# MalvinaNikandrou/mafed

Hardware: AMD Instinct MI355X
Metric: train samples/sec VLPythia-410M+MAFED, 256img+32txt tok, bs=32, 1/2/4/8 GPU (higher is better)
Workload: dtype bf16; 1 GPU; VLPythia-410m + MAFED distill step (student fwd+bwd, frozen-teacher fwd, replay CE, 23-layer per-modality MSE, clip 2.0, AdamW), 256 img + 32 txt tokens; global_batch=32, per_gpu_batch=32, seq_len=288, parallelism=dp1, random_init_weights=True

## Files before the change

mafed_amd/csrc/attn_mfma.hip:

```cpp
#include <type_traits>

#include "attn.h"

namespace mafed {

namespace {

typedef __attribute__((address_space(3))) bf16x4* lds_bf16x4_ptr;

template <int D>
__device__ __forceinline__ int swz(int row) {
  if (D == 64) return ((row >> 1) & 3) << 1;
  if (D == 128) return (row & 7) << 1;
  return ((row & 7) << 1) | ((row >> 3) & 1);
}
template <int D>
__device__ __forceinline__ int tile_off(int row, int chunk) {
  if (D == 64) return row * 128 + ((chunk ^ swz<64>(row)) << 4);
  if (D == 128) return row * 256 + ((chunk ^ swz<128>(row)) << 4);
  return row * 512 + ((chunk ^ (((row & 7) << 1) | ((row >> 3) & 1))) << 4);
}

__device__ __forceinline__ void unpack8(const uint4& v, float (&f)[8]) {
  f[0] = __uint_as_float(v.x << 16); f[1] = __uint_as_float(v.x & 0xffff0000u);
// ... 683 lines not shown
  extern __shared__ __attribute__((aligned(16))) char lds[];
  constexpr int NTH = NW * 64;
  const int tid = threadIdx.x, lane = tid & 63;
  const int wave = __builtin_amdgcn_readfirstlane(tid >> 6);
  const int S = sh.S, H = sh.H, rot = sh.rot, P = sh.P, T = sh.T;
  const int h = blockIdx.x, b = blockIdx.y;
  const int nrows = (S + 31) / 32 * 32;
  char* kimg = lds;
  char* vimg = lds + nrows * D * 2;
  float* kbias = reinterpret_cast<float*>(lds + 2 * nrows * D * 2);
  float* red = kbias + 2 * nrows;
  if (bsum && tid < D) red[tid] = 0.f;
  const int64_t rstride = (int64_t)H * 3 * D;
  const bf16_t* qb = qkv + ((int64_t)b * S * H + h) * 3 * D;
  const bf16_t* kb = qb + D;
  const bf16_t* vb = qb + 2 * D;
  const int64_t ostride = (int64_t)H * D;
  const bf16_t* ob = out + (int64_t)b * S * ostride + (int64_t)h * D;
  const bf16_t* dob = dout + (int64_t)b * S * ostride + (int64_t)h * D;
  const float* Lrow = lse + ((int64_t)b * H + h) * S;
  const int nslices = (S + 15) / 16;
  const int hc = rot >> 4, items = S * hc;
  dma_rows<D, NW>(kimg, kb, rstride, nrows, S, wave, lane);
  dma_rows<D, NW>(vimg, vb, rstride, nrows, S, wave, lane);
  RotPre pre[2];
#pragma unroll
  for (int u = 0; u < 2; ++u)
    if (tid + NTH * u < items) rot_pre_load(pre[u], tid + NTH * u, hc, rot, rc, rs);
  for (int k = tid; k < nrows; k += NTH) kbias[k] = key_ok(am, b, k, P, T, S) ? 0.f : -INFINITY;
  constexpr bool PREFETCH = NW == 4;
  ColRaw<D> qraw, doraw, oraw;
  float Lnext = 0.f;
  if (PREFETCH) {
    const int s0 = nslices - 1 - snake<NW>(wave, 0);
    if (s0 >= 0) {
      col_raw_issue<D, true>(qraw, qb, rstride, s0 * 16, S, rot, rc, rs, lane);
      col_raw_issue<D, false>(doraw, dob, ostride, s0 * 16, S, 0, rc, rs, lane);
      col_raw_issue<D, false>(oraw, ob, ostride, s0 * 16, S, 0, rc, rs, lane);
      const int q = s0 * 16 + (lane & 15);
      Lnext = q < S ? Lrow[q] : 0.f;
    }
  }
  wait_vm0();
  __syncthreads();
  rot_fix_rows<D, NTH>(kimg, items, hc, rot, rc, rs, pre, tid);
  __syncthreads();
  const int g = lane >> 4;
  const float scale = rsqrtf((float)D);
  const float scale2 = scale * MAFED_LOG2E;
  for (int t = 0;; ++t) {
    const int slice = nslices - 1 - snake<NW>(wave, t);
    if (slice < 0) break;
    const int q0 = slice * 16;
    const int myq = q0 + (lane & 15);
    if (!PREFETCH) {
      col_raw_issue<D, true>(qraw, qb, rstride, q0, S, rot, rc, rs, lane);
      col_raw_issue<D, false>(doraw, dob, ostride, q0, S, 0, rc, rs, lane);
      col_raw_issue<D, false>(oraw, ob, ostride, q0, S, 0, rc, rs, lane);
      Lnext = myq < S ? Lrow[myq] : 0.f;
    }
    bf16x8 qf[D / 32], dof[D / 32];
    col_raw_finish<D, true>(qf, qraw, q0, S, rot, lane);
    col_raw_finish<D, false>(dof, doraw, q0, S, 0, lane);
    const float L2 = Lnext * MAFED_LOG2E;
    float dl = 0.f;
    {
      bf16x8 of[D / 32];
      col_raw_finish<D, false>(of, oraw, q0, S, 0, lane);
      const int nxt = nslices - 1 - snake<NW>(wave, t + 1);
      if (PREFETCH && nxt >= 0) {
        col_raw_issue<D, true>(qraw, qb, rstride, nxt * 16, S, rot, rc, rs, lane);
        col_raw_issue<D, false>(doraw, dob, ostride, nxt * 16, S, 0, rc, rs, lane);
        col_raw_issue<D, false>(oraw, ob, ostride, nxt * 16, S, 0, rc, rs, lane);
        const int q = nxt * 16 + (lane & 15);
        Lnext = q < S ? Lrow[q] : 0.f;
      }
#pragma unroll
      for (int ks = 0; ks < D / 32; ++ks)
#pragma unroll
        for (int e = 0; e < 8; ++e) dl += (float)dof[ks][e] * (float)of[ks][e];
      dl = col_sum_sw(dl);
    }
    if (myq < S && g == 0) delta[((int64_t)b * H + h) * S + myq] = dl;
    f32x4 dq[D / 16];
#pragma unroll
    for (int i = 0; i < D / 16; ++i) dq[i] = (f32x4){0.f, 0.f, 0.f, 0.f};
    const int last_kt = (q0 + 15) / 64;
    auto tile = [&](const int kt, const int nj, auto mask_tag) {
      constexpr bool MASK = decltype(mask_tag)::value;
      f32x4 ds[4];
#pragma unroll
      for (int j = 0; j < 4; ++j) {
        ds[j] = (f32x4){0.f, 0.f, 0.f, 0.f};
        if (!MASK || j < nj) {
          f32x4 s = (f32x4){0.f, 0.f, 0.f, 0.f}, dp = (f32x4){0.f, 0.f, 0.f, 0.f};
#pragma unroll
          for (int ks = 0; ks < D / 32; ++ks) {
            s = __builtin_amdgcn_mfma_f32_16x16x32_bf16(frag_row<D>(kimg, kt * 4 + j, ks, lane), qf[ks], s, 0, 0, 0);
            dp = __builtin_amdgcn_mfma_f32_16x16x32_bf16(frag_row<D>(vimg, kt * 4 + j, ks, lane), dof[ks], dp, 0, 0, 0);
          }
          if (MASK) {
            const float4 kb4 = *reinterpret_cast<const float4*>(kbias + kt * 64 + j * 16 + 4 * g);
            const float kbv[4] = {kb4.x, kb4.y, kb4.z, kb4.w};
#pragma unroll
            for (int r = 0; r < 4; ++r) {
              const int key = kt * 64 + j * 16 + 4 * g + r;
              float x = s[r] * scale2 - L2 + kbv[r];
              x = key > myq ? -INFINITY : x;
              ds[j][r] = __builtin_amdgcn_exp2f(x) * (dp[r] - dl) * scale;
            }
          } else {
#pragma unroll
            for (int r = 0; r < 4; ++r) ds[j][r] = __builtin_amdgcn_exp2f(s[r] * scale2 - L2) * (dp[r] - dl) * scale;
          }
        }
      }
      const bf16x8 d0 = pack_acc(ds[0], ds[1]);
#pragma unroll
      for (int dt = 0; dt < D / 16; ++dt) dq[dt] = __builtin_amdgcn_mfma_f32_16x16x32_bf16(frag_tr<D>(kimg, dt, kt * 2, lane), d0, dq[dt], 0, 0, 0);
      if (!MASK || nj > 2) {
        const bf16x8 d1 = pack_acc(ds[2], ds[3]);
#pragma unroll
        for (int dt = 0; dt < D / 16; ++dt)
          dq[dt] = __builtin_amdgcn_mfma_f32_16x16x32_bf16(frag_tr<D>(kimg, dt, kt * 2 + 1, lane), d1, dq[dt], 0, 0, 0);
      }
    };
    const int kt_plain = last_kt < P / 64 ? last_kt : P / 64;
    for (int kt = 0; kt < kt_plain; ++kt) tile(kt, 4, std::false_type{});
    for (int kt = kt_plain; kt <= last_kt; ++kt) tile(kt, kt == last_kt ? ((q0 + 15 - kt * 64) >> 4) + 1 : 4, std::true_type{});
    bf16_t* dqp = dqkv + ((int64_t)b * S * H + h) * 3 * D + (int64_t)myq * rstride;
    store_grad_unrot<D>(dqp, dq, rot, rc, rs, myq, lane, myq < S);
    if (bsum) {
#pragma unroll
      for (int dt = 0; dt < D / 16; ++dt)
#pragma unroll
        for (int r = 0; r < 4; ++r) {
          const float v = row16_sum(myq < S ? dq[dt][r] : 0.f);
          if ((lane & 15) == 0) atomicAdd(red + dt * 16 + 4 * g + r, v);
        }
    }
  }
  if (bsum) {
    __syncthreads();
    if (tid < D) atomicAdd(bsum + (int64_t)h * 3 * D + tid, red[tid]);
  }
}

template <int D, int NW = 4>
__global__ __launch_bounds__(NW * 64, (D == 64 ? 2 : 1) * NW / 4) void attn_bwd_dkv_res_kernel(const bf16_t* __restrict__ qkv, const bf16_t* __restrict__ dout,
                                                               const float* __restrict__ lse, const float* __restrict__ delta, AttnShape sh,
                                                               const float* __restrict__ rc, const float* __restrict__ rs,
                                                               const int64_t* __restrict__ am, bf16_t* __restrict__ dqkv,
                                                               float* __restrict__ bsum) {
  extern __shared__ __attribute__((aligned(16))) char lds[];
  constexpr int NTH = NW * 64;
  const int tid = threadIdx.x, lane = tid & 63;
  const int wave = __builtin_amdgcn_readfirstlane(tid >> 6);
  const int S = sh.S, H = sh.H, rot = sh.rot, P = sh.P, T = sh.T;
  const int h = blockIdx.x, b = blockIdx.y;
  const int nrows = (S + 31) / 32 * 32;
  char* qimg = lds;
  char* doimg = lds + nrows * D * 2;
  float* L2s = reinterpret_cast<float*>(lds + 2 * nrows * D * 2);
  float* Ds = L2s + nrows;
  float* red = Ds + nrows;
  if (bsum && tid < 2 * D) red[tid] = 0.f;
  const int64_t rstride = (int64_t)H * 3 * D;
  const bf16_t* qb = qkv + ((int64_t)b * S * H + h) * 3 * D;
  const bf16_t* kb = qb + D;
  const bf16_t* vb = qb + 2 * D;
  const int64_t ostride = (int64_t)H * D;
  const bf16_t* dob = dout + (int64_t)b * S * ostride + (int64_t)h * D;
  const float* Lrow = lse + ((int64_t)b * H + h) * S;
  const float* Drow = delta + ((int64_t)b * H + h) * S;
  const int nslices = (S + 15) / 16;
  const int hc = rot >> 4, items = S * hc;
  dma_rows<D, NW>(qimg, qb, rstride, nrows, S, wave, lane);
  dma_rows<D, NW>(doimg, dob, ostride, nrows, S, wave, lane);
  RotPre pre[2];
#pragma unroll
  for (int u = 0; u < 2; ++u)
    if (tid + NTH * u < items) rot_pre_load(pre[u], tid + NTH * u, hc, rot, rc, rs);
  for (int q = tid; q < nrows; q += NTH) {
    L2s[q] = q < S ? Lrow[q] * MAFED_LOG2E : INFINITY;
    Ds[q] = q < S ? Drow[q] : 0.f;
  }
  ColRaw<D> kraw, vraw;
  {
    const int s0 = snake<NW>(wave, 0);
    if (s0 < nslices) {
      col_raw_issue<D, true>(kraw, kb, rstride, s0 * 16, S, rot, rc, rs, lane);
      col_raw_issue<D, false>(vraw, vb, rstride, s0 * 16, S, 0, rc, rs, lane);
    }
  }
  wait_vm0();
  __syncthreads();
  rot_fix_rows<D, NTH>(qimg, items, hc, rot, rc, rs, pre, tid);
  __syncthreads();
  const int g = lane >> 4;
  const float scale = rsqrtf((float)D);
  const float scale2 = scale * MAFED_LOG2E;
  const int nqt = (nrows + 63) / 64;
  for (int t = 0;; ++t) {
    const int slice = snake<NW>(wave, t);
    if (slice >= nslices) break;
    const int k0 = slice * 16;
    const int mykey = k0 + (lane & 15);
    const int mykey_eff = key_ok(am, b, mykey, P, T, S) ? mykey : 0x7fffffff;
    bf16x8 kf[D / 32], vf[D / 32];
    col_raw_finish<D, true>(kf, kraw, k0, S, rot, lane);
    col_raw_finish<D, false>(vf, vraw, k0, S, 0, lane);
    {
      const int nxt = snake<NW>(wave, t + 1);
      if (nxt < nslices) {
        col_raw_issue<D, true>(kraw, kb, rstride, nxt * 16, S, rot, rc, rs, lane);
        col_raw_issue<D, false>(vraw, vb, rstride, nxt * 16, S, 0, rc, rs, lane);
      }
    }
    f32x4 dk[D / 16], dv[D / 16];
#pragma unroll
    for (int i = 0; i < D / 16; ++i) { dk[i] = (f32x4){0.f, 0.f, 0.f, 0.f}; dv[i] = (f32x4){0.f, 0.f, 0.f, 0.f}; }
    const int qt0 = k0 / 64;
    const bool text_keys = k0 + 15 >= P;
    auto tile = [&](const int qt, const int jlo, const int jhi, auto edge_tag) {
      constexpr bool EDGE = decltype(edge_tag)::value;
      f32x4 p[4], ds[4];
#pragma unroll
      for (int j = 0; j < 4; ++j) {
        p[j] = (f32x4){0.f, 0.f, 0.f, 0.f};
        ds[j] = (f32x4){0.f, 0.f, 0.f, 0.f};
        if (!EDGE || (j >= jlo && j < jhi)) {
          f32x4 s = (f32x4){0.f, 0.f, 0.f, 0.f}, dp = (f32x4){0.f, 0.f, 0.f, 0.f};
#pragma unroll
          for (int ks = 0; ks < D / 32; ++ks) {
            s = __builtin_amdgcn_mfma_f32_16x16x32_bf16(frag_row<D>(qimg, qt * 4 + j, ks, lane), kf[ks], s, 0, 0, 0);
            dp = __builtin_amdgcn_mfma_f32_16x16x32_bf16(frag_row<D>(doimg, qt * 4 + j, ks, lane), vf[ks], dp, 0, 0, 0);
          }
          const float4 L4 = *reinterpret_cast<const float4*>(L2s + qt * 64 + j * 16 + 4 * g);
          const float4 D4 = *reinterpret_cast<const float4*>(Ds + qt * 64 + j * 16 + 4 * g);
          const float Lv[4] = {L4.x, L4.y, L4.z, L4.w}, Dv[4] = {D4.x, D4.y, D4.z, D4.w};
#pragma unroll
          for (int r = 0; r < 4; ++r) {
            float x = s[r] * scale2 - Lv[r];
            if (EDGE) {
              const int q = qt * 64 + j * 16 + 4 * g + r;
              x = mykey_eff > q ? -INFINITY : x;
            }
            const float pv = __builtin_amdgcn_exp2f(x);
            p[j][r] = pv;
            ds[j][r] = pv * (dp[r] - Dv[r]) * scale;
          }
        }
      }
      if (!EDGE || jlo < 2) {
        const bf16x8 p0 = pack_acc(p[0], p[1]), d0 = pack_acc(ds[0], ds[1]);
#pragma unroll
        for (int dt = 0; dt < D / 16; ++dt) {
          dv[dt] = __builtin_amdgcn_mfma_f32_16x16x32_bf16(frag_tr<D>(doimg, dt, qt * 2, lane), p0, dv[dt], 0, 0, 0);
          dk[dt] = __builtin_amdgcn_mfma_f32_16x16x32_bf16(frag_tr<D>(qimg, dt, qt * 2, lane), d0, dk[dt], 0, 0, 0);
        }
      }
      if (!EDGE || jhi > 2) {
        const bf16x8 p1 = pack_acc(p[2], p[3]), d1 = pack_acc(ds[2], ds[3]);
#pragma unroll
        for (int dt = 0; dt < D / 16; ++dt) {
          dv[dt] = __builtin_amdgcn_mfma_f32_16x16x32_bf16(frag_tr<D>(doimg, dt, qt * 2 + 1, lane), p1, dv[dt], 0, 0, 0);
          dk[dt] = __builtin_amdgcn_mfma_f32_16x16x32_bf16(frag_tr<D>(qimg, dt, qt * 2 + 1, lane), d1, dk[dt], 0, 0, 0);
        }
      }
    };
    const int nfull = nrows / 64;
    for (int qt = qt0; qt < nqt; ++qt) {
      const int jlo = qt == qt0 ? (k0 - qt * 64) >> 4 : 0;
      const int jhi = (nrows - qt * 64) >> 4 < 4 ? (nrows - qt * 64) >> 4 : 4;
      if (qt == qt0 || text_keys || qt >= nfull) tile(qt, jlo, jhi, std::true_type{});
      else tile(qt, 0, 4, std::false_type{});
    }
    bf16_t* dkp = dqkv + ((int64_t)b * S * H + h) * 3 * D + (int64_t)mykey * rstride + D;
    store_grad_unrot<D>(dkp, dk, rot, rc, rs, mykey, lane, mykey < S);
    if (mykey < S) {
      bf16_t* dvp = dkp + D;
#pragma unroll
      for (int dt = 0; dt < D / 16; ++dt) store4(dvp + dt * 16 + 4 * g, make_float4(dv[dt][0], dv[dt][1], dv[dt][2], dv[dt][3]));
    }
    if (bsum) {
#pragma unroll
      for (int dt = 0; dt < D / 16; ++dt)
#pragma unroll
        for (int r = 0; r < 4; ++r) {
          const float vk = row16_sum(mykey < S ? dk[dt][r] : 0.f), vv = row16_sum(mykey < S ? dv[dt][r] : 0.f);
          if ((lane & 15) == 0) {
            atomicAdd(red + dt * 16 + 4 * g + r, vk);
            atomicAdd(red + D + dt * 16 + 4 * g + r, vv);
          }
        }
    }
  }
  if (bsum) {
    __syncthreads();
    if (tid < 2 * D) atomicAdd(bsum + (int64_t)h * 3 * D + D + tid, red[tid]);
  }
}

static double attn_fwd_flops(const AttnShape& sh) { return 4.0 * sh.D * ((double)sh.S * (sh.S + 1) / 2.0) * sh.H * sh.B; }

static bool attn_resident_fits(const AttnShape& sh, size_t* bytes) {
  const size_t nrows = (size_t)(sh.S + 31) / 32 * 32;
  *bytes = nrows * sh.D * 2 * 2 + nrows * 4 * 2 + (size_t)sh.D * 4 * 2;
  return sh.D <= 128 && *bytes <= 160 * 1024;
}
static int g_attn_variant = 0;

template <typename K>
static void set_lds_attr(K kfn, size_t bytes) {
  (void)hipFuncSetAttribute((const void*)kfn, hipFuncAttributeMaxDynamicSharedMemorySize, (int)bytes);
}

int attn_mfma_fwd_launch(const void* qkv, const AttnShape& sh, const float* rc, const float* rs, const int64_t* am, void* out, float* lse,
                         hipStream_t st) {
  size_t bytes;
  if (g_attn_variant != 1 && attn_resident_fits(sh, &bytes)) {
    dim3 grid(sh.H, sh.B), block(attn_fwd_waves<64>() * 64);
    if (!sh.causal) {
      if (sh.D != 64) { set_error("attn_fwd (bidirectional, bf16): head_dim %d has no MFMA kernel (CLIP towers use 64)", sh.D); return MAFED_EINVAL; }
      set_lds_attr(attn_fwd_res_kernel<64, false>, bytes);
      launch(K_ATTN_FWD, 2.0 * attn_fwd_flops(sh), attn_fwd_res_kernel<64, false>, grid, block, bytes, st, (const bf16_t*)qkv, sh, rc, rs, am,
             (bf16_t*)out, lse);
      return MAFED_OK;
    }
    if (sh.D == 64) {
      set_lds_attr(attn_fwd_res_kernel<64>, bytes);
      launch(K_ATTN_FWD, attn_fwd_flops(sh), attn_fwd_res_kernel<64>, grid, block, bytes, st, (const bf16_t*)qkv, sh, rc, rs, am, (bf16_t*)out, lse);
    } else {
      set_lds_attr(attn_fwd_res_kernel<128>, bytes);
      launch(K_ATTN_FWD, attn_fwd_flops(sh), attn_fwd_res_kernel<128>, grid, dim3(attn_fwd_waves<128>() * 64), bytes, st, (const bf16_t*)qkv, sh, rc, rs, am, (bf16_t*)out, lse);
    }
    return MAFED_OK;
  }
  if (!sh.causal) { set_error("attn_fwd (bidirectional, bf16): S=%d D=%d does not fit the resident kernel", sh.S, sh.D); return MAFED_EINVAL; }
  dim3 grid((sh.S + 63) / 64, sh.H, sh.B), block(256);
  const size_t tb = (size_t)2 * 64 * sh.D * 2;
#define MAFED_FWD_TILED(DD)                                                                                                       \
  do {                                                                                                                            \
    set_lds_attr(attn_fwd_mfma_kernel<DD>, tb);                                                                                   \
    launch(K_ATTN_FWD, attn_fwd_flops(sh), attn_fwd_mfma_kernel<DD>, grid, block, tb, st, (const bf16_t*)qkv, sh, rc, rs, am, (bf16_t*)out, lse);                    \
  } while (0)
  if (sh.D == 64) MAFED_FWD_TILED(64);
  else if (sh.D == 128) MAFED_FWD_TILED(128);
  else MAFED_FWD_TILED(256);
#undef MAFED_FWD_TILED
  return MAFED_OK;
}

int attn_mfma_bwd_launch(const void* qkv, const void* out, const void* dout, const float* lse, const AttnShape& sh, const float* rc,
                         const float* rs, const int64_t* am, void* dqkv, float* delta, float* colsum, bool* colsum_done, hipStream_t st) {
  size_t bytes;
  *colsum_done = false;
  if (g_attn_variant != 1 && attn_resident_fits(sh, &bytes)) {
    dim3 grid(sh.H, sh.B), block(256);
    if (sh.D == 64) {
      set_lds_attr(attn_bwd_dq_res_kernel<64>, bytes);
      set_lds_attr(attn_bwd_dkv_res_kernel<64>, bytes);
      launch(K_ATTN_BWD_DQ, attn_fwd_flops(sh), attn_bwd_dq_res_kernel<64>, grid, block, bytes, st, (const bf16_t*)qkv, (const bf16_t*)out, (const bf16_t*)dout, lse, sh, rc, rs, am,
                                                             (bf16_t*)dqkv, delta, colsum);
      launch(K_ATTN_BWD_DKV, attn_fwd_flops(sh), attn_bwd_dkv_res_kernel<64>, grid, block, bytes, st, (const bf16_t*)qkv, (const bf16_t*)dout, lse, delta, sh, rc, rs, am, (bf16_t*)dqkv, colsum);
    } else {
      set_lds_attr(attn_bwd_dq_res_kernel<128>, bytes);
      set_lds_attr(attn_bwd_dkv_res_kernel<128>, bytes);
      launch(K_ATTN_BWD_DQ, attn_fwd_flops(sh), attn_bwd_dq_res_kernel<128>, grid, block, bytes, st, (const bf16_t*)qkv, (const bf16_t*)out, (const bf16_t*)dout, lse, sh, rc, rs, am,
                                                              (bf16_t*)dqkv, delta, colsum);
      launch(K_ATTN_BWD_DKV, attn_fwd_flops(sh), attn_bwd_dkv_res_kernel<128>, grid, block, bytes, st, (const bf16_t*)qkv, (const bf16_t*)dout, lse, delta, sh, rc, rs, am, (bf16_t*)dqkv, colsum);
    }
    *colsum_done = colsum != nullptr;
    return MAFED_OK;
  }
  dim3 grid((sh.S + 63) / 64, sh.H, sh.B), block(256);
  const size_t tb = (size_t)2 * 64 * sh.D * 2, tb2 = tb + 2 * 64 * 4;
#define MAFED_BWD_TILED(DD)                                                                                                       \
  do {                                                                                                                            \
    set_lds_attr(attn_bwd_dq_mfma_kernel<DD>, tb);                                                                                \
    set_lds_attr(attn_bwd_dkv_mfma_kernel<DD>, tb2);                                                                              \
    launch(K_ATTN_BWD_DQ, attn_fwd_flops(sh), attn_bwd_dq_mfma_kernel<DD>, grid, block, tb, st, (const bf16_t*)qkv, (const bf16_t*)out, (const bf16_t*)dout, lse, sh, rc, rs, am, \
                                                         (bf16_t*)dqkv, delta);                                                  \
    launch(K_ATTN_BWD_DKV, attn_fwd_flops(sh), attn_bwd_dkv_mfma_kernel<DD>, grid, block, tb2, st, (const bf16_t*)qkv, (const bf16_t*)dout, lse, delta, sh, rc, rs, am,   \
                                                           (bf16_t*)dqkv);                                                       \
  } while (0)
  if (sh.D == 64) MAFED_BWD_TILED(64);
  else if (sh.D == 128) MAFED_BWD_TILED(128);
  else MAFED_BWD_TILED(256);
#undef MAFED_BWD_TILED
  return MAFED_OK;
}

void attn_mfma_set_variant(int v) { g_attn_variant = v; }


}
```

Before: 1006 samples/s.

## Fuse attention backward dQ and dK/dV into one LDS-resident kernel

Adds a single backward attention kernel for head_dim 64. It loads Q, K, V and dO once into LDS per (head, batch), computes delta in-kernel, and interleaves key-slice (dK/dV) and query-slice (dQ) work items across 12 waves. This replaces the two separate resident kernels, which each reloaded tiles and recomputed S and dP. The cost is a larger LDS footprint, fewer blocks per CU, and S and dP still being recomputed in both the key and query items.

```diff
diff --git a/mafed_amd/csrc/attn_mfma.hip b/mafed_amd/csrc/attn_mfma.hip
--- a/mafed_amd/csrc/attn_mfma.hip
+++ b/mafed_amd/csrc/attn_mfma.hip
@@ -1009,12 +1009,256 @@
   }
 }
 
+constexpr int kFusedWaves = 12;
+
+__global__ __launch_bounds__(kFusedWaves * 64, kFusedWaves / 4) void attn_bwd_fused_kernel(const bf16_t* __restrict__ qkv, const bf16_t* __restrict__ out,
+                                                                             const bf16_t* __restrict__ dout, const float* __restrict__ lse, AttnShape sh,
+                                                                             const float* __restrict__ rc, const float* __restrict__ rs,
+                                                                             const int64_t* __restrict__ am, bf16_t* __restrict__ dqkv,
+                                                                             float* __restrict__ delta, float* __restrict__ bsum) {
+  constexpr int D = 64, NW = kFusedWaves, NTH = NW * 64;
+  extern __shared__ __attribute__((aligned(16))) char lds[];
+  const int tid = threadIdx.x, lane = tid & 63;
+  const int wave = __builtin_amdgcn_readfirstlane(tid >> 6);
+  const int S = sh.S, H = sh.H, rot = sh.rot, P = sh.P, T = sh.T;
+  const int h = blockIdx.x, b = blockIdx.y;
+  const int nrows = (S + 31) / 32 * 32;
+  char* qimg = lds;
+  char* kimg = lds + 1 * nrows * D * 2;
+  char* vimg = lds + 2 * nrows * D * 2;
+  char* doimg = lds + 3 * nrows * D * 2;
+  float* kbias = reinterpret_cast<float*>(lds + 4 * nrows * D * 2);
+  float* L2s = kbias + nrows;
+  float* Ds = L2s + nrows;
+  float* red = Ds + nrows;
+  if (bsum && tid < 3 * D) red[tid] = 0.f;
+  const int64_t rstride = (int64_t)H * 3 * D;
+  const bf16_t* qb = qkv + ((int64_t)b * S * H + h) * 3 * D;
+  const bf16_t* kb = qb + D;
+  const bf16_t* vb = qb + 2 * D;
+  const int64_t ostride = (int64_t)H * D;
+  const bf16_t* ob = out + (int64_t)b * S * ostride + (int64_t)h * D;
+  const bf16_t* dob = dout + (int64_t)b * S * ostride + (int64_t)h * D;
+  const float* Lrow = lse + ((int64_t)b * H + h) * S;
+  const int nslices = (S + 15) / 16;
+  const int hc = rot >> 4, items = S * hc;
+  dma_rows<D, NW>(qimg, qb, rstride, nrows, S, wave, lane);
+  dma_rows<D, NW>(doimg, dob, ostride, nrows, S, wave, lane);
+  dma_rows<D, NW>(kimg, kb, rstride, nrows, S, wave, lane);
+  dma_rows<D, NW>(vimg, vb, rstride, nrows, S, wave, lane);
+  RotPre pre[2];
+#pragma unroll
+  for (int u = 0; u < 2; ++u)
+    if (tid + NTH * u < items) rot_pre_load(pre[u], tid + NTH * u, hc, rot, rc, rs);
+  for (int k = tid; k < nrows; k += NTH) {
+    kbias[k] = key_ok(am, b, k, P, T, S) ? 0.f : -INFINITY;
+    L2s[k] = k < S ? Lrow[k] * MAFED_LOG2E : INFINITY;
+  }
+  for (int r0 = 0; r0 < nrows; r0 += NTH / 8) {
+    const int row = r0 + (tid >> 3), ch = tid & 7;
+    float dl = 0.f;
+    if (row < S) {
+      float fo[8], fd[8];
+      unpack8(*reinterpret_cast<const uint4*>(ob + (int64_t)row * ostride + ch * 8), fo);
+      unpack8(*reinterpret_cast<const uint4*>(dob + (int64_t)row * ostride + ch * 8), fd);
+#pragma unroll
+      for (int e = 0; e < 8; ++e) dl = fmaf(fd[e], fo[e], dl);
+    }
+    dl += __shfl_xor(dl, 1, 64);
+    dl += __shfl_xor(dl, 2, 64);
+    dl += __shfl_xor(dl, 4, 64);
+    if (row < nrows && ch == 0) {
+      Ds[row] = dl;
+      if (row < S) delta[((int64_t)b * H + h) * S + row] = dl;
+    }
+  }
+  wait_vm0();
+  __syncthreads();
+  rot_fix_rows<D, NTH>(qimg, items, hc, rot, rc, rs, pre, tid);
+  rot_fix_rows<D, NTH>(kimg, items, hc, rot, rc, rs, pre, tid);
+  __syncthreads();
+  const int g = lane >> 4;
+  const float scale = rsqrtf((float)D);
+  const float scale2 = scale * MAFED_LOG2E;
+  const int nqt = (nrows + 63) / 64;
+  const int nfull = nrows / 64;
+  bf16_t* dqkv_bh = dqkv + ((int64_t)b * S * H + h) * 3 * D;
+
+  auto key_item = [&](const int slice) {
+    const int k0 = slice * 16;
+    const int mykey = k0 + (lane & 15);
+    const int mykey_eff = key_ok(am, b, mykey, P, T, S) ? mykey : 0x7fffffff;
+    bf16x8 kf[D / 32], vf[D / 32];
+#pragma unroll
+    for (int ks = 0; ks < D / 32; ++ks) {
+      kf[ks] = frag_row<D>(kimg, slice, ks, lane);
+      vf[ks] = frag_row<D>(vimg, slice, ks, lane);
+    }
+    f32x4 dk[D / 16], dv[D / 16];
+#pragma unroll
+    for (int i = 0; i < D / 16; ++i) { dk[i] = (f32x4){0.f, 0.f, 0.f, 0.f}; dv[i] = (f32x4){0.f, 0.f, 0.f, 0.f}; }
+    const int qt0 = k0 / 64;
+    const bool text_keys = k0 + 15 >= P;
+    auto tile = [&](const int qt, const int jlo, const int jhi, auto edge_tag) {
+      constexpr bool EDGE = decltype(edge_tag)::value;
+#pragma nounroll
+      for (int hh = 0; hh < 2; ++hh) {
+        if (EDGE && (2 * hh + 1 < jlo || 2 * hh >= jhi)) continue;
+        f32x4 p[2], ds[2];
+#pragma unroll
+        for (int jj = 0; jj < 2; ++jj) {
+          const int j = 2 * hh + jj;
+          p[jj] = (f32x4){0.f, 0.f, 0.f, 0.f};
+          ds[jj] = (f32x4){0.f, 0.f, 0.f, 0.f};
+          if (!EDGE || (j >= jlo && j < jhi)) {
+            f32x4 s = (f32x4){0.f, 0.f, 0.f, 0.f}, dp = (f32x4){0.f, 0.f, 0.f, 0.f};
+#pragma unroll
+            for (int ks = 0; ks < D / 32; ++ks) {
+              s = __builtin_amdgcn_mfma_f32_16x16x32_bf16(frag_row<D>(qimg, qt * 4 + j, ks, lane), kf[ks], s, 0, 0, 0);
+              dp = __builtin_amdgcn_mfma_f32_16x16x32_bf16(frag_row<D>(doimg, qt * 4 + j, ks, lane), vf[ks], dp, 0, 0, 0);
+            }
+            const float4 L4 = *reinterpret_cast<const float4*>(L2s + qt * 64 + j * 16 + 4 * g);
+            const float4 D4 = *reinterpret_cast<const float4*>(Ds + qt * 64 + j * 16 + 4 * g);
+            const float Lv[4] = {L4.x, L4.y, L4.z, L4.w}, Dv[4] = {D4.x, D4.y, D4.z, D4.w};
+#pragma unroll
+            for (int r = 0; r < 4; ++r) {
+              float x = s[r] * scale2 - Lv[r];
+              if (EDGE) {
+                const int q = qt * 64 + j * 16 + 4 * g + r;
+                x = mykey_eff > q ? -INFINITY : x;
+              }
+              const float pv = __builtin_amdgcn_exp2f(x);
+              p[jj][r] = pv;
+              ds[jj][r] = pv * (dp[r] - Dv[r]) * scale;
+            }
+          }
+        }
+        const bf16x8 p0 = pack_acc(p[0], p[1]), d0 = pack_acc(ds[0], ds[1]);
+#pragma unroll
+        for (int dt = 0; dt < D / 16; ++dt) {
+          dv[dt] = __builtin_amdgcn_mfma_f32_16x16x32_bf16(frag_tr<D>(doimg, dt, qt * 2 + hh, lane), p0, dv[dt], 0, 0, 0);
+          dk[dt] = __builtin_amdgcn_mfma_f32_16x16x32_bf16(frag_tr<D>(qimg, dt, qt * 2 + hh, lane), d0, dk[dt], 0, 0, 0);
+        }
+      }
+    };
+    for (int qt = qt0; qt < nqt; ++qt) {
+      const int jlo = qt == qt0 ? (k0 - qt * 64) >> 4 : 0;
+      const int jhi = (nrows - qt * 64) >> 4 < 4 ? (nrows - qt * 64) >> 4 : 4;
+      if (qt == qt0 || text_keys || qt >= nfull) tile(qt, jlo, jhi, std::true_type{});
+      else tile(qt, 0, 4, std::false_type{});
+    }
+    bf16_t* dkp = dqkv_bh + (int64_t)mykey * rstride + D;
+    store_grad_unrot<D>(dkp, dk, rot, rc, rs, mykey, lane, mykey < S);
+    if (mykey < S) {
+      bf16_t* dvp = dkp + D;
+#pragma unroll
+      for (int dt = 0; dt < D / 16; ++dt) store4(dvp + dt * 16 + 4 * g, make_float4(dv[dt][0], dv[dt][1], dv[dt][2], dv[dt][3]));
+    }
+    if (bsum) {
+#pragma unroll
+      for (int dt = 0; dt < D / 16; ++dt)
+#pragma unroll
+        for (int r = 0; r < 4; ++r) {
+          const float vk = row16_sum(mykey < S ? dk[dt][r] : 0.f), vv = row16_sum(mykey < S ? dv[dt][r] : 0.f);
+          if ((lane & 15) == 0) {
+            atomicAdd(red + D + dt * 16 + 4 * g + r, vk);
+            atomicAdd(red + 2 * D + dt * 16 + 4 * g + r, vv);
+          }
+        }
+    }
+  };
+
+  auto query_item = [&](const int slice) {
+    const int q0 = slice * 16;
+    const int myq = q0 + (lane & 15);
+    bf16x8 qf[D / 32], dof[D / 32];
+#pragma unroll
+    for (int ks = 0; ks < D / 32; ++ks) {
+      qf[ks] = frag_row<D>(qimg, slice, ks, lane);
+      dof[ks] = frag_row<D>(doimg, slice, ks, lane);
+    }
+    const float L2 = L2s[myq], dl = Ds[myq];
+    f32x4 dq[D / 16];
+#pragma unroll
+    for (int i = 0; i < D / 16; ++i) dq[i] = (f32x4){0.f, 0.f, 0.f, 0.f};
+    const int last_kt = (q0 + 15) / 64;
+    auto tile = [&](const int kt, const int nj, auto mask_tag) {
+      constexpr bool MASK = decltype(mask_tag)::value;
+#pragma nounroll
+      for (int hh = 0; hh < 2; ++hh) {
+        if (MASK && 2 * hh >= nj) break;
+        f32x4 ds[2];
+#pragma unroll
+        for (int jj = 0; jj < 2; ++jj) {
+          const int j = 2 * hh + jj;
+          ds[jj] = (f32x4){0.f, 0.f, 0.f, 0.f};
+          if (!MASK || j < nj) {
+            f32x4 s = (f32x4){0.f, 0.f, 0.f, 0.f}, dp = (f32x4){0.f, 0.f, 0.f, 0.f};
+#pragma unroll
+            for (int ks = 0; ks < D / 32; ++ks) {
+              s = __builtin_amdgcn_mfma_f32_16x16x32_bf16(frag_row<D>(kimg, kt * 4 + j, ks, lane), qf[ks], s, 0, 0, 0);
+              dp = __builtin_amdgcn_mfma_f32_16x16x32_bf16(frag_row<D>(vimg, kt * 4 + j, ks, lane), dof[ks], dp, 0, 0, 0);
+            }
+            if (MASK) {
+              const float4 kb4 = *reinterpret_cast<const float4*>(kbias + kt * 64 + j * 16 + 4 * g);
+              const float kbv[4] = {kb4.x, kb4.y, kb4.z, kb4.w};
+#pragma unroll
+              for (int r = 0; r < 4; ++r) {
+                const int key = kt * 64 + j * 16 + 4 * g + r;
+                float x = s[r] * scale2 - L2 + kbv[r];
+                x = key > myq ? -INFINITY : x;
+                ds[jj][r] = __builtin_amdgcn_exp2f(x) * (dp[r] - dl) * scale;
+              }
+            } else {
+#pragma unroll
+              for (int r = 0; r < 4; ++r) ds[jj][r] = __builtin_amdgcn_exp2f(s[r] * scale2 - L2) * (dp[r] - dl) * scale;
+            }
+          }
+        }
+        const bf16x8 d0 = pack_acc(ds[0], ds[1]);
+#pragma unroll
+        for (int dt = 0; dt < D / 16; ++dt)
+          dq[dt] = __builtin_amdgcn_mfma_f32_16x16x32_bf16(frag_tr<D>(kimg, dt, kt * 2 + hh, lane), d0, dq[dt], 0, 0, 0);
+      }
+    };
+    const int kt_plain = last_kt < P / 64 ? last_kt : P / 64;
+    for (int kt = 0; kt < kt_plain; ++kt) tile(kt, 4, std::false_type{});
+    for (int kt = kt_plain; kt <= last_kt; ++kt) tile(kt, kt == last_kt ? ((q0 + 15 - kt * 64) >> 4) + 1 : 4, std::true_type{});
+    store_grad_unrot<D>(dqkv_bh + (int64_t)myq * rstride, dq, rot, rc, rs, myq, lane, myq < S);
+    if (bsum) {
+#pragma unroll
+      for (int dt = 0; dt < D / 16; ++dt)
+#pragma unroll
+        for (int r = 0; r < 4; ++r) {
+          const float v = row16_sum(myq < S ? dq[dt][r] : 0.f);
+          if ((lane & 15) == 0) atomicAdd(red + dt * 16 + 4 * g + r, v);
+        }
+    }
+  };
+
+  for (int t = 0;; ++t) {
+    const int item = snake<NW>(wave, t);
+    if (item >= 2 * nslices) break;
+    if (item & 1) query_item(nslices - 1 - (item >> 1));
+    else key_item(item >> 1);
+  }
+  if (bsum) {
+    __syncthreads();
+    if (tid < 3 * D) atomicAdd(bsum + (int64_t)h * 3 * D + tid, red[tid]);
+  }
+}
+
 static double attn_fwd_flops(const AttnShape& sh) { return 4.0 * sh.D * ((double)sh.S * (sh.S + 1) / 2.0) * sh.H * sh.B; }
 
 static bool attn_resident_fits(const AttnShape& sh, size_t* bytes) {
   const size_t nrows = (size_t)(sh.S + 31) / 32 * 32;
   *bytes = nrows * sh.D * 2 * 2 + nrows * 4 * 2 + (size_t)sh.D * 4 * 2;
   return sh.D <= 128 && *bytes <= 160 * 1024;
+}
+static bool attn_fused_bwd_fits(const AttnShape& sh, size_t* bytes) {
+  const size_t nrows = (size_t)(sh.S + 31) / 32 * 32;
+  *bytes = nrows * sh.D * 2 * 4 + nrows * 4 * 3 + (size_t)sh.D * 4 * 3;
+  return sh.D == 64 && *bytes <= 160 * 1024;
 }
 static int g_attn_variant = 0;
 
@@ -1063,6 +1307,13 @@
                          const float* rs, const int64_t* am, void* dqkv, float* delta, float* colsum, bool* colsum_done, hipStream_t st) {
   size_t bytes;
   *colsum_done = false;
+  if (g_attn_variant == 0 && attn_fused_bwd_fits(sh, &bytes)) {
+    set_lds_attr(attn_bwd_fused_kernel, bytes);
+    launch(K_ATTN_BWD_DQ, 2.0 * attn_fwd_flops(sh), attn_bwd_fused_kernel, dim3(sh.H, sh.B), dim3(kFusedWaves * 64), bytes, st, (const bf16_t*)qkv,
+           (const bf16_t*)out, (const bf16_t*)dout, lse, sh, rc, rs, am, (bf16_t*)dqkv, delta, colsum);
+    *colsum_done = colsum != nullptr;
+    return MAFED_OK;
+  }
   if (g_attn_variant != 1 && attn_resident_fits(sh, &bytes)) {
     dim3 grid(sh.H, sh.B), block(256);
     if (sh.D == 64) {
```

Result: no change. 1007 samples/s (median of 6 runs) (+0.2%).
